# amcpherson/defuse

Hardware: AMD Instinct MI355X
Metric: split-read DP aligns/sec (higher is better)
Workload: dtype int16

## Files before the change

defuse_amd/csrc/dsa_kernels.hpp:

```cpp
#pragma once
#include <hip/hip_runtime.h>
#include <stdint.h>

#include "../../include/defuse_dsa.h"
#include "dsa_diag.hpp"
#include "dsa_tile.hpp"

namespace dsa {

constexpr int W = TILE_W;
constexpr int WAVE = 64;
constexpr int WG_WAVES = 4;
constexpr int WG_LANES = WG_WAVES * WAVE;
constexpr uint32_t REF_PAD16 = 0x00AAu;
constexpr uint32_t ROW_PAD16 = 0x0055u;

constexpr int NCLS = 5;
constexpr int NCOMBO = NCLS * NCLS;
constexpr int TROW = W + 4;
#ifndef FILL_PF
#define FILL_PF 2
#endif
constexpr int GMAX = 4;
constexpr int TGROUP = NCOMBO * TROW;
// ... 700 lines not shown
            ++gi;
        }
        tasks[tb + t] = rt;
    }
}

struct HitCursor {
    int k0, k1;
    int row0, row1;
    uint32_t t0, t1;
    uint64_t valid0, valid1;
};
__device__ __forceinline__ KeptRow kept_row(const KeptRow* __restrict__ kr, const uint64_t* kc, int k)
{
    if (kc != nullptr && k < KCACHE) return __builtin_bit_cast(KeptRow, kc[k * WG_LANES]);
    return kr[k];
}
__device__ __forceinline__ void cursor_next0(HitCursor& hc, const KeptRow* __restrict__ kr, const uint64_t* kc, int n_kept, bool has0)
{
    hc.row0 = -1;
    if (has0 && hc.k0 < n_kept) {
        const KeptRow r = kept_row(kr, kc, hc.k0);
        hc.row0 = r.a;
        hc.t0 = (uint32_t)(r.m1 + 2 * r.a) + BIAS16;
    }
}
__device__ __forceinline__ void cursor_next1(HitCursor& hc, const KeptRow* __restrict__ kr, const uint64_t* kc, int lq, bool has1)
{
    hc.row1 = -1;
    if (has1 && hc.k1 >= 0) {
        const KeptRow r = kept_row(kr, kc, hc.k1);
        hc.row1 = lq - r.a;
        hc.t1 = (uint32_t)(r.m2 + 2 * (lq - r.a)) + BIAS16;
    }
}
__device__ __forceinline__ HitCursor cursor_init(const KeptRow* __restrict__ kr, const uint64_t* kc, int n_kept, int lq,
                                                 bool has0, bool has1, int nv0, int nv1)
{
    HitCursor hc;
    hc.k0 = 0;
    hc.k1 = n_kept - 1;
    hc.t0 = hc.t1 = 0;
    hc.valid0 = nv0 >= W ? ~0ull : ((1ull << (nv0 > 0 ? nv0 : 0)) - 1ull);
    hc.valid1 = nv1 >= W ? ~0ull : ((1ull << (nv1 > 0 ? nv1 : 0)) - 1ull);
    cursor_next0(hc, kr, kc, n_kept, has0);
    cursor_next1(hc, kr, kc, lq, has1);
    return hc;
}

constexpr uint32_t NO_TARGET16 = 0x7F00u;
template <int WT>
__device__ __forceinline__ void equal_columns(const uint32_t (&X)[WT], uint32_t target2, uint64_t& m0, uint64_t& m1)
{
    uint32_t hit[W / 16];
    const uint32_t below = target2 - 0x00010001u;
#pragma unroll
    for (int q = 0; q < W / 16; ++q) {
        uint32_t acc = 0;
#pragma unroll
        for (int k = 15; k >= 0; --k) {
            const int i = 16 * q + k;
            if (i >= WT) continue;
            const uint32_t c = below + drift2(i);
            typedef unsigned short us2 __attribute__((ext_vector_type(2)));
            const uint32_t y = __builtin_bit_cast(uint32_t, __builtin_elementwise_sub_sat(__builtin_bit_cast(us2, X[i]), __builtin_bit_cast(us2, c)));
            asm("v_lshl_or_b32 %0, %0, 1, %1" : "+v"(acc) : "v"(y));
        }
        hit[q] = acc;
    }
    const uint32_t lo_a = (hit[0] & 0xFFFFu) | (hit[1] << 16), lo_b = (hit[2] & 0xFFFFu) | (hit[3] << 16);
    const uint32_t hi_a = (hit[0] >> 16) | (hit[1] & 0xFFFF0000u), hi_b = (hit[2] >> 16) | (hit[3] & 0xFFFF0000u);
    m0 = (uint64_t)lo_a | ((uint64_t)lo_b << 32);
    m1 = (uint64_t)hi_a | ((uint64_t)hi_b << 32);
}

template <int WT>
__device__ __forceinline__ void record_hits(const uint32_t (&X)[WT], int j, int lq, const KeptRow* __restrict__ kr,
                                            const uint64_t* kc, int n_kept, bool has0, bool has1, HitCursor& hc,
                                            uint64_t* __restrict__ masks, uint32_t mask_begin)
{
    const bool hit0 = hc.row0 == j, hit1 = hc.row1 == j;
    if (!(hit0 || hit1)) return;
    uint64_t m0, m1;
    equal_columns(X, (hit0 ? hc.t0 : NO_TARGET16) | ((hit1 ? hc.t1 : NO_TARGET16) << 16), m0, m1);
    if (hit0) {
        masks[((uint64_t)mask_begin + hc.k0) * 2] = m0 & hc.valid0;
        ++hc.k0;
        cursor_next0(hc, kr, kc, n_kept, has0);
    }
    if (hit1) {
        masks[((uint64_t)mask_begin + hc.k1) * 2 + 1] = m1 & hc.valid1;
        --hc.k1;
        cursor_next1(hc, kr, kc, lq, has1);
    }
}

__device__ __forceinline__ int64_t count_one_tile_pair(const uint64_t* mk, int n_kept)
{
    int64_t n = 0;
    for (int k = 0; k < n_kept; ++k) {
        const uint64_t m0 = mk[2 * k], m1 = mk[2 * k + 1];
        if (k == 0) {
            n += (int64_t)__builtin_popcountll(m0) * __builtin_popcountll(m1);
            continue;
        }
        for (uint64_t r0 = m0; r0; r0 &= r0 - 1)
            for (uint64_t r1 = m1; r1; r1 &= r1 - 1) {
                const int i1 = __builtin_ctzll(r0), i2 = __builtin_ctzll(r1);
                bool dup = false;
                for (int k2 = 0; k2 < k && !dup; ++k2) dup = ((mk[2 * k2] >> i1) & 1ull) && ((mk[2 * k2 + 1] >> i2) & 1ull);
                n += dup ? 0 : 1;
            }
    }
    return n;
}

template <bool SPLIT, int WT>
__device__ __forceinline__ void replay_fast_wg(uint32_t* T, FinishLds* fl, const WgView& wgi, const FinishBufs& fb,
                                               const uint32_t* __restrict__ refcodes, const uint32_t* __restrict__ rowcodes,
                                               const uint32_t* __restrict__ bnd, const Geom& g)
{
    const KeptRow* __restrict__ kept = fb.kept;
    uint64_t* __restrict__ masks = fb.masks;
    bool any = false;
    for (int k = 0; k < wgi.n_groups; ++k) any |= fl->tile[k] >= 0;
    if (!uniform(any)) return;
    build_tables<SPLIT, WT>(T, wgi.n_groups, [&](int gi, int i, uint32_t& q0, uint32_t& q1) {
        const int key = fl->tile[gi];
        q0 = q1 = REF_PAD16;
        if (key >= 0) {
            const int c0 = key >> 8, c1 = key & 0xFF;
            const uint32_t* rc = refcodes + (int64_t)group_fusion(wgi, gi) * g.lrp;
            if (c0 != NO_CHUNK) q0 = rc[c0 * W + i] & 0xFFFFu;
            if (c1 != NO_CHUNK) q1 = rc[c1 * W + i] >> 16;
        }
    });
    for (int e = threadIdx.x; e < 258; e += WG_LANES) fl->hist[e] = 0;
    __syncthreads();
    int my_key = 256, my_rank = 0;
    {
        const LaneInfo mine = fl->info[threadIdx.x];
        if (mine.last_row & TASK_FAST) my_key = mine.key_group & 0xFF;
        my_rank = atomicAdd(&fl->hist[my_key], 1);
    }
    __syncthreads();
    if (threadIdx.x == 0) {
        int run = 0;
        for (int e = 0; e < 257; ++e) {
            const int n = fl->hist[e];
            fl->hist[e] = run;
            run += n;
        }
    }
    __syncthreads();
    fl->order[fl->hist[my_key] + my_rank] = (unsigned short)threadIdx.x;
    __syncthreads();

    const int src = fl->order[threadIdx.x];
    const LaneInfo li = fl->info[src];
    const int64_t p = (int64_t)blockIdx.x * WG_LANES + src;
    const int lane = (int)(p & 63);
    const int64_t w = p >> 6;
    const bool has = (li.last_row & TASK_FAST) != 0;
    const int R = has ? (li.last_row & TASK_ROW) : 0;
    int Rw = R;
#pragma unroll
    for (int d = 32; d >= 1; d >>= 1) Rw = max(Rw, __shfl_xor(Rw, d, 64));
    Rw = uniform(Rw);
    if (Rw == 0) return;
    const bool has0 = has && li.c0 != NO_CHUNK, has1 = has && li.c1 != NO_CHUNK;
    const int c0 = has0 ? li.c0 : 0, c1 = has1 ? li.c1 : 0;
    const uint32_t* tb = T + (li.key_group >> 8) * (SPLIT ? TGROUP_SPLIT : TGROUP);
    const int64_t wr = w < g.n_waves ? w : (int64_t)blockIdx.x * WG_WAVES;
    const uint4* rows4 = reinterpret_cast<const uint4*>(rowcodes + wr * g.lq1 * WAVE) + lane;
    const uint4* bi0 = reinterpret_cast<const uint4*>(bnd + (wr * g.nch + (c0 - 1)) * g.lq1 * WAVE) + lane;
    const uint4* bi1 = reinterpret_cast<const uint4*>(bnd + (wr * g.nch + (c1 - 1)) * g.lq1 * WAVE) + lane;
    const KeptRow* kr = kept + li.kept_begin;
    const uint64_t* kc = fl->kc + src;
    const int lq = li.lq;
    const int n_kept = has ? li.n_kept : 0;
    HitCursor hc = cursor_init(kr, kc, n_kept, lq, has0, has1, li.nv0, li.nv1);
    const int stop0 = c0 > 0 ? load_tstop(fb.tstop + wr * g.nch + (c0 - 1)) : 0;
    const int stop1 = c1 > 0 ? load_tstop(fb.tstop + wr * g.nch + (c1 - 1)) : 0;

    uint32_t X[WT];
#pragma unroll
    for (int i = 0; i < WT; ++i) X[i] = BIAS2 + drift2(i);
    const uint4 bias4 = make_uint4(BIAS2, BIAS2, BIAS2, BIAS2);
    uint32_t bprev = BIAS2;
    const int ngq = (Rw >> 2) + 1;
    auto boundary = [&](int gq) -> uint4 {
        uint4 x0 = bias4, x1 = bias4;
        if (gq < stop0) x0 = load_group(bi0 + (int64_t)gq * WAVE);
        if (gq < stop1) x1 = load_group(bi1 + (int64_t)gq * WAVE);
        return make_uint4((x0.x & 0xFFFFu) | (x1.x & 0xFFFF0000u), (x0.y & 0xFFFFu) | (x1.y & 0xFFFF0000u),
                          (x0.z & 0xFFFFu) | (x1.z & 0xFFFF0000u), (x0.w & 0xFFFFu) | (x1.w & 0xFFFF0000u));
    };
    uint4 rc_n = rows4[0];
    uint4 b_n = boundary(0);
    for (int gq = 0; gq < ngq; ++gq) {
        const uint4 rc = rc_n, b = b_n;
        const int gn = gq + 1 < ngq ? gq + 1 : gq;
        rc_n = rows4[(int64_t)gn * WAVE];
        b_n = boundary(gn);
        const uint32_t rcv[4] = {rc.x, rc.y, rc.z, rc.w}, bv[4] = {b.x, b.y, b.z, b.w};
#pragma unroll
        for (int sidx = 0; sidx < 4; ++sidx) {
            const int j = 4 * gq + sidx;
            const uint32_t bcur = bv[sidx];
            if (j >= 1 && j <= Rw) {
                const uint4* trow = reinterpret_cast<const uint4*>(tb + (rcv[sidx] & 0xFFu) * TROW);
                auto table4 = [&](int q) -> uint4 {
                    if (SPLIT) return split_terms(tb, (rcv[sidx] >> 16) & 0xFu, (rcv[sidx] >> 20) & 0xFu, q);
                    return trow[q];
                };
                uint4 v = table4(0);
                uint32_t a = bprev + v.x;
                uint32_t up = bcur - TWO2;
#pragma unroll
                for (int q = 0; q < WT / 4; ++q) {
                    uint4 vn = v;
                    if (q + 1 < WT / 4) vn = table4(q + 1);
                    uint32_t an;
                    an = X[4 * q + 0] + v.y;
                    X[4 * q + 0] = max3(a, X[4 * q + 0], up);
                    a = an;
                    an = X[4 * q + 1] + v.z;
                    X[4 * q + 1] = max3(a, X[4 * q + 1], X[4 * q + 0]);
                    a = an;
                    an = X[4 * q + 2] + v.w;
                    X[4 * q + 2] = max3(a, X[4 * q + 2], X[4 * q + 1]);
                    a = an;
                    an = X[4 * q + 3] + vn.x;
                    X[4 * q + 3] = max3(a, X[4 * q + 3], X[4 * q + 2]);
                    a = an;
                    up = X[4 * q + 3];
                    v = vn;
                }
                record_hits(X, j, lq, kr, kc, n_kept, has0, has1, hc, masks, li.mask_begin);
            }
            bprev = bcur;
        }
    }
    if (has && !has0)
        for (int k = 0; k < n_kept; ++k) masks[((uint64_t)li.mask_begin + k) * 2] = 0;
    if (has && !has1)
        for (int k = 0; k < n_kept; ++k) masks[((uint64_t)li.mask_begin + k) * 2 + 1] = 0;
    if (has && (li.last_row & TASK_ONLY) && p < g.n_pairs)
        fb.rec_count[g.orig ? g.orig[p] : p] = count_one_tile_pair(masks + (uint64_t)li.mask_begin * 2, n_kept);
}

template <bool MASKED, int WT>
__device__ __forceinline__ int sweep_tile_generic(const uint32_t (&r)[WT], const uint4* __restrict__ rows4,
                                                  const uint4* __restrict__ bi4, uint4* __restrict__ cm4,
                                                  uint4* __restrict__ bo4, int lq, bool first, int nv0, int nv1,
                                                  int lq_lane, int slack, int l_in, int stop_prev, int& last_bnd)
{
    uint32_t X[WT];
#pragma unroll
    for (int i = 0; i < WT; ++i) X[i] = BIAS2 + drift2(i);
    const uint4 bias4 = make_uint4(BIAS2, BIAS2, BIAS2, BIAS2);
    uint32_t bprev = BIAS2;
    const int ngq = (lq >> 2) + 1;
    uint4 rc_n = rows4[0];
    uint4 b_n = first ? bias4 : bi4[0];
    last_bnd = 0;
    int gq = 0;
    for (; gq < ngq; ++gq) {
        const uint4 rc = rc_n, b = b_n;
        const int gn = gq + 1 < ngq ? gq + 1 : gq;
        rc_n = rows4[(int64_t)gn * WAVE];
        b_n = (!first && gn < stop_prev) ? bi4[(int64_t)gn * WAVE] : bias4;
        const uint32_t rcv[4] = {rc.x, rc.y, rc.z, rc.w}, bv[4] = {b.x, b.y, b.z, b.w};
        uint32_t cmv[4] = {BIAS2, BIAS2, BIAS2, BIAS2}, bov[4] = {BIAS2, BIAS2, BIAS2, BIAS2};
        bool alive = false;
#pragma unroll
        for (int sidx = 0; sidx < 4; ++sidx) {
            const int j = 4 * gq + sidx;
            if (j >= 1 && j <= lq) {
                row_step(X, r, rcv[sidx], bprev, bv[sidx]);
                cmv[sidx] = tile_row_max<MASKED>(X, nv0, nv1);
                bov[sidx] = X[WT - 1] - drift2(WT - 1);
                const int thr = 4 * j - slack + (int)BIAS16;
                const bool in_read = j <= lq_lane;
                alive |= in_read && ((int)(cmv[sidx] & 0xFFFFu) >= thr || (int)(cmv[sidx] >> 16) >= thr);
                if (in_read && ((int)(bov[sidx] & 0xFFFFu) >= thr || (int)(bov[sidx] >> 16) >= thr)) last_bnd = j;
            }
            bprev = bv[sidx];
        }
        cm4[(int64_t)gq * WAVE] = make_uint4(cmv[0], cmv[1], cmv[2], cmv[3]);
        bo4[(int64_t)gq * WAVE] = make_uint4(bov[0], bov[1], bov[2], bov[3]);
        if (DIAG_PRUNE && 4 * gq + 3 > l_in && __builtin_amdgcn_ballot_w64(alive) == 0) { ++gq; break; }
    }
    return gq;
}

__device__ __forceinline__ void max4(uint4& m, const uint4& v)
{
    m.x = max2(m.x, v.x);
    m.y = max2(m.y, v.y);
    m.z = max2(m.z, v.z);
    m.w = max2(m.w, v.w);
}
template <bool WIDE>
__device__ __forceinline__ void reduce_row_max(const uint32_t* __restrict__ cmax, uint32_t* __restrict__ rmax,
                                               const int32_t* tstop, const TileStops& stops,
                                               const Geom& g, int w, int lane, int nch_wave, int lq)
{
    const int ngq = (lq >> 2) + 1;
    const uint4 dead4 = make_uint4(BIAS2, BIAS2, BIAS2, BIAS2);
    uint4* out = reinterpret_cast<uint4*>(rmax + (int64_t)w * g.lq1 * WAVE) + lane;
    const uint4* src = reinterpret_cast<const uint4*>(cmax + (int64_t)w * g.nch * g.lq1 * WAVE) + lane;
    const int64_t cstride = (int64_t)(g.lq1 >> 2) * WAVE;
    constexpr int NC = 8;
    if (nch_wave <= NC) {
        for (int gq = 0; gq < ngq; ++gq) {
            uint4 v[NC];
#pragma unroll
            for (int c = 0; c < NC; ++c)
                if (gq < stops.v[c]) v[c] = src[c * cstride + (int64_t)gq * WAVE];
            uint4 m = dead4;
#pragma unroll
            for (int c = 0; c < NC; ++c)
                if (gq < stops.v[c]) max4(m, v[c]);
            out[(int64_t)gq * WAVE] = m;
        }
        return;
    }
    if (WIDE && nch_wave <= 2 * NC) {
        int stop_hi[NC];
#pragma unroll
        for (int c = 0; c < NC; ++c) stop_hi[c] = NC + c < nch_wave ? uniform(load_tstop(tstop + (int64_t)w * g.nch + NC + c)) : 0;
        for (int gq = 0; gq < ngq; ++gq) {
            uint4 v[NC], u[NC];
#pragma unroll
            for (int c = 0; c < NC; ++c) {
                if (gq < stops.v[c]) v[c] = src[c * cstride + (int64_t)gq * WAVE];
                if (gq < stop_hi[c]) u[c] = src[(NC + c) * cstride + (int64_t)gq * WAVE];
            }
            uint4 m = dead4;
#pragma unroll
            for (int c = 0; c < NC; ++c) {
                if (gq < stops.v[c]) max4(m, v[c]);
                if (gq < stop_hi[c]) max4(m, u[c]);
            }
            out[(int64_t)gq * WAVE] = m;
        }
        return;
    }
    for (int gq = 0; gq < ngq; ++gq) {
        uint4 m = dead4;
        for (int c = 0; c < nch_wave; ++c)
            if (gq < uniform(load_tstop(tstop + (int64_t)w * g.nch + c))) max4(m, src[c * cstride + (int64_t)gq * WAVE]);
        out[(int64_t)gq * WAVE] = m;
    }
}

template <int WT>
__global__ __launch_bounds__(WG_LANES) void k_fill_generic(const dsa_pair* __restrict__ pairs,
                                                           const dsa_fusion* __restrict__ fusions,
                                                           const uint8_t* __restrict__ wg_tier,
                                                           const uint32_t* __restrict__ refcodes,
                                                           const uint8_t* __restrict__ read_bytes,
                                                           uint32_t* __restrict__ rowcodes,
                                                           const int32_t* __restrict__ min_score_tab,
                                                           uint32_t* __restrict__ bnd, uint32_t* __restrict__ cmax,
                                                           uint32_t* __restrict__ rmax,
                                                           FinishBufs fb, Geom g)
{
    __shared__ FinishLds fl;
    if (wg_tier[blockIdx.x] != TIER_GENERIC) return;
    if (threadIdx.x == 0) atomicAdd(&fb.ctr->fill_wgs[FILL_WGS_GENERIC], 1u);
    const int w = __builtin_amdgcn_readfirstlane((int)(blockIdx.x * WG_WAVES + (threadIdx.x >> 6)));
    TileStops stops = {};
    if (w < g.n_waves) {
        const int lane = threadIdx.x & 63;
        const int64_t p = min((int64_t)w * WAVE + lane, g.n_pairs - 1);
        const bool in_batch = (int64_t)w * WAVE + lane < g.n_pairs;
        const int f = pairs[p].fusion_idx;
        const dsa_fusion fu = fusions[f];
        auto wave_max = [](int v) {
#pragma unroll
            for (int d = 32; d >= 1; d >>= 1) v = max(v, __shfl_xor(v, d, 64));
            return uniform(v);
        };
        WaveInfo wi;
        wi.lq_max = wave_max(in_batch ? (int)pairs[p].read_len : 0);
        wi.nch_max = wave_max(in_batch ? max(cdiv_dev(fu.ref0_len, WT), cdiv_dev(fu.ref1_len, WT)) : 0);
        (void)pack_rows_wave<0>(read_bytes, pairs, rowcodes, nullptr, g, w, lane, wi.lq_max);
        const uint32_t* rc = refcodes + (int64_t)f * g.lrp;
        const uint4* rows4 = reinterpret_cast<const uint4*>(rowcodes + (int64_t)w * g.lq1 * WAVE) + lane;
        int lq_lane = 0, slack = 0;
        if (in_batch) {
            lq_lane = pairs[p].read_len;
            slack = 2 * lq_lane - max(min_score_tab[lq_lane], pair_bound(pairs[p]));
        }
        int l_in = wave_max(lq_lane > 0 ? min(slack >> 2, lq_lane) : 0);
        int stop_prev = 0;

        for (int c = 0; c < wi.nch_max; ++c) {
            uint32_t r[WT];
#pragma unroll
            for (int i = 0; i < WT; ++i) r[i] = rc[c * W + i];
            const int nv0 = fu.ref0_len - c * WT, nv1 = fu.ref1_len - c * WT;
            uint4* cm4 = reinterpret_cast<uint4*>(cmax + ((int64_t)w * g.nch + c) * g.lq1 * WAVE) + lane;
            uint4* bo4 = reinterpret_cast<uint4*>(bnd + ((int64_t)w * g.nch + c) * g.lq1 * WAVE) + lane;
            const uint4* bi4 = reinterpret_cast<const uint4*>(bnd + ((int64_t)w * g.nch + (c - 1)) * g.lq1 * WAVE) + lane;
            int last_bnd, stop;
            if (__builtin_amdgcn_ballot_w64(nv0 < WT || nv1 < WT) == 0)
                stop = sweep_tile_generic<false, WT>(r, rows4, bi4, cm4, bo4, wi.lq_max, c == 0, nv0, nv1, lq_lane, slack, l_in, stop_prev, last_bnd);
            else
                stop = sweep_tile_generic<true, WT>(r, rows4, bi4, cm4, bo4, wi.lq_max, c == 0, nv0, nv1, lq_lane, slack, l_in, stop_prev, last_bnd);
            if (lane == 0) fb.tstop[(int64_t)w * g.nch + c] = stop;
            stop_prev = stop;
#pragma unroll
            for (int k = 0; k < 8; ++k)
                if (k == c) stops.v[k] = stop;
            l_in = wave_max(last_bnd);
        }
        __builtin_amdgcn_fence(__ATOMIC_RELEASE, "workgroup");
        reduce_row_max<false>(cmax, rmax, fb.tstop, stops, g, w, lane, wi.nch_max, wi.lq_max);
    }
    WgView wgi = {};
    wgi.list = nullptr;
    combine_wg<false, WT>(pairs, fusions, cmax, rmax, stops, min_score_tab, wgi, 0, false, &fl, fb, g);
}

template <int NW, bool SPLIT, bool LAST>
__device__ __forceinline__ int sweep_tile_fast(const uint32_t* __restrict__ tb, const uint32_t* __restrict__ rows1, const uint4* __restrict__ bi4,
                                               uint4* __restrict__ cm4, uint4* __restrict__ bo4, bool first_tile, int lq_max, int lq_lane,
                                               uint32_t thr0, int l_in, int stop_prev, int& last_bnd, const Geom& g, int tile)
{
    static_assert(NW % 4 == 0 && NW / 4 > FILL_PF && NW <= W, "table reads in flight");
    (void)g; (void)tile;
    uint32_t X[NW];
#pragma unroll
    for (int i = 0; i < NW; ++i) X[i] = BIAS2 + drift2(i);
    const uint4 bias4 = make_uint4(BIAS2, BIAS2, BIAS2, BIAS2);
    uint32_t bprev = BIAS2;
    const int ngq = (lq_max >> 2) + 1;
    uint32_t rc_n = rows1[0];
    uint4 b_n = first_tile ? bias4 : bi4[0];
    last_bnd = 0;
    int gq = 0;
    int n_gap_groups = 0;
    for (; gq < ngq; ++gq) {
        const uint32_t rc = rc_n;
        const uint4 b = b_n;
        const int gn = gq + 1 < ngq ? gq + 1 : gq;
        rc_n = rows1[(int64_t)gn * WAVE];
        b_n = bias4;
        if (gn < stop_prev) b_n = load_group(bi4 + (int64_t)gn * WAVE);
        const uint32_t bv[4] = {b.x, b.y, b.z, b.w};
        uint32_t cmv[4] = {BIAS2, BIAS2, BIAS2, BIAS2}, bov[4] = {BIAS2, BIAS2, BIAS2, BIAS2};
        uint32_t alive_bits = 0;
#pragma unroll
        for (int sidx = 0; sidx < 4; ++sidx) {
            const int j = 4 * gq + sidx;
            const uint32_t bcur = bv[sidx];
            if (j >= 1 && j <= lq_max) {
                if constexpr (SPLIT) {
                    const uint32_t k1 = (rc >> (8 * sidx)) & 0xFu, k2 = (rc >> (8 * sidx + 4)) & 0xFu;
                    uint4 v = split_terms(tb, k1, k2, 0);
                    uint32_t a = bprev + v.x;
                    uint32_t up = bcur - TWO2;
#pragma unroll
                    for (int q = 0; q < NW / 4; ++q) {
                        uint4 vn = v;
                        if (q + 1 < NW / 4) vn = split_terms(tb, k1, k2, q + 1);
                        uint32_t an;
                        an = X[4 * q + 0] + v.y;
                        X[4 * q + 0] = max3(a, X[4 * q + 0], up);
                        a = an;
                        an = X[4 * q + 1] + v.z;
                        X[4 * q + 1] = max3(a, X[4 * q + 1], X[4 * q + 0]);
                        a = an;
                        an = X[4 * q + 2] + v.w;
                        X[4 * q + 2] = max3(a, X[4 * q + 2], X[4 * q + 1]);
                        a = an;
                        an = X[4 * q + 3] + vn.x;
                        X[4 * q + 3] = max3(a, X[4 * q + 3], X[4 * q + 2]);
                        a = an;
                        up = X[4 * q + 3];
                        v = vn;
                    }
                } else {
                    const uint4* trow = reinterpret_cast<const uint4*>(tb + ((rc >> (8 * sidx)) & 0xFFu) * TROW);
                    uint4 vq[FILL_PF + 1];
#pragma unroll
                    for (int k = 0; k <= FILL_PF; ++k) vq[k] = trow[k];
                    uint32_t a = bprev + vq[0].x;
                    uint32_t up = bcur - TWO2;
#pragma unroll
                    for (int q = 0; q < NW / 4; ++q) {
                        const uint4 v = vq[0];
#pragma unroll
                        for (int k = 0; k < FILL_PF; ++k) vq[k] = vq[k + 1];
                        if (q + 1 + FILL_PF < NW / 4) vq[FILL_PF] = trow[q + 1 + FILL_PF];
                        const uint4 vn = vq[0];
                        uint32_t an;
                        an = X[4 * q + 0] + v.y;
                        X[4 * q + 0] = max3(a, X[4 * q + 0], up);
                        a = an;
                        an = X[4 * q + 1] + v.z;
                        X[4 * q + 1] = max3(a, X[4 * q + 1], X[4 * q + 0]);
                        a = an;
                        an = X[4 * q + 2] + v.w;
                        X[4 * q + 2] = max3(a, X[4 * q + 2], X[4 * q + 1]);
                        a = an;
                        an = X[4 * q + 3] + vn.x;
                        X[4 * q + 3] = max3(a, X[4 * q + 3], X[4 * q + 2]);
                        a = an;
                        up = X[4 * q + 3];
                    }
                }
                {
                    uint32_t acc0 = BIAS2, acc1 = BIAS2;
#pragma unroll
                    for (int i = 0; i < NW; i += 4) {
                        acc0 = max3(acc0, X[i] - drift2(i), X[i + 1] - drift2(i + 1));
                        acc1 = max3(acc1, X[i + 2] - drift2(i + 2), X[i + 3] - drift2(i + 3));
                    }
                    cmv[sidx] = max2(acc0, acc1);
                }
                const uint32_t tm2 = thr_of_row(thr0, j, j <= lq_lane);
                alive_bits |= pk_max_u16(cmv[sidx], tm2) ^ tm2;
                if (!LAST) {
                    bov[sidx] = X[NW - 1] - drift2(NW - 1);
                    if ((pk_max_u16(bov[sidx], tm2) ^ tm2) != 0u) last_bnd = j;
                }
            }
            bprev = bcur;
        }
        const bool alive = alive_bits != 0u;
        cm4[(int64_t)gq * WAVE] = make_uint4(cmv[0], cmv[1], cmv[2], cmv[3]);
        if (!LAST) bo4[(int64_t)gq * WAVE] = make_uint4(bov[0], bov[1], bov[2], bov[3]);
        if (DIAG_PRUNE && __builtin_amdgcn_ballot_w64(alive) == 0) {
            if (4 * gq + 3 > l_in) { ++gq; break; }
            if (DIAG_GAP_SKIP) {
                int g2 = gq + 1;
                bool resume = false;
                uint4 bb = b_n;
                uint32_t in_prev = bv[3];
                for (; g2 < ngq; ++g2) {
                    if (g2 > gq + 1) {
                        bb = bias4;
                        if (g2 < stop_prev) bb = load_group(bi4 + (int64_t)g2 * WAVE);
                    }
                    const uint32_t bbv[5] = {in_prev, bb.x, bb.y, bb.z, bb.w};
                    uint32_t in_bits = 0;
#pragma unroll
                    for (int sidx = 0; sidx < 5; ++sidx) {
                        const int j = 4 * g2 + sidx - 1;
                        const uint32_t tm2 = thr_of_row(thr0, j, j <= lq_lane);
                        in_bits |= pk_max_u16(bbv[sidx], tm2) ^ tm2;
                    }
                    if (__builtin_amdgcn_ballot_w64(in_bits != 0u) != 0) { resume = true; break; }
                    cm4[(int64_t)g2 * WAVE] = bias4;
                    if (!LAST) bo4[(int64_t)g2 * WAVE] = bias4;
                    in_prev = bb.w;
                    if (4 * g2 + 3 > l_in) { ++g2; break; }
                }
                n_gap_groups += g2 - (gq + 1);
                if (!resume) { gq = g2; break; }
#pragma unroll
                for (int i = 0; i < NW; ++i) X[i] = BIAS2 + drift2(i);
                bprev = in_prev;
                b_n = bb;
                rc_n = rows1[(int64_t)g2 * WAVE];
                gq = g2 - 1;
            }
        }
    }
    if ((threadIdx.x & 63) == 0) {
        DSA_STAT_ADD(g, DS_GAP_GROUPS, n_gap_groups);
        DSA_STAT_ADD(g, DS_GROUPS_SKIPPED, ngq - gq);
        DSA_STAT_ADD(g, DS_GROUPS, ngq);
        DSA_STAT_ADD(g, DS_TILE_GROUPS + (tile < DS_TILE_SLOTS ? tile : DS_TILE_SLOTS - 1), gq - n_gap_groups);
    }
    return gq;
}

__host__ __device__ constexpr int tier_of(int n_groups) { return n_groups <= GMAX ? 0 : n_groups <= GSPLIT ? 1 : 2; }
#ifndef DSA_FAST_WGS
#define DSA_FAST_WGS 4
#endif
template <int TIER, bool WIDE, int WT>
__global__ __launch_bounds__(WG_LANES, TIER == 2 ? 2 : DSA_FAST_WGS) void k_fill_fast(const dsa_pair* __restrict__ pairs,
                                                           uint8_t* __restrict__ wg_tier,
                                                           const uint32_t* __restrict__ refcodes,
                                                           const uint8_t* __restrict__ read_bytes,
                                                           uint32_t* __restrict__ rowcodes, uint32_t* __restrict__ row_bytes,
                                                           const int32_t* __restrict__ min_score_tab,
                                                           const dsa_fusion* __restrict__ fusions,
                                                           uint32_t* __restrict__ bnd, uint32_t* __restrict__ cmax,
                                                           uint32_t* __restrict__ rmax,
                                                           FinishBufs fb, Geom g)
{
    constexpr bool SPLIT = TIER > 0;
    __shared__ __attribute__((aligned(16))) uint32_t T[TIER == 2 ? GSPLIT2 * TGROUP_SPLIT : GMAX * TGROUP];
    __shared__ int s_nch, s_exotic;
    __shared__ FinishLds fl;
    __shared__ WgGroupsLds gl;
    if (TIER != 0 && wg_tier[blockIdx.x] != TIER) return;
    const int w = __builtin_amdgcn_readfirstlane((int)(blockIdx.x * WG_WAVES + (threadIdx.x >> 6)));
    const bool live = w < g.n_waves;
    const int lane = threadIdx.x & 63;
    const int64_t p = (int64_t)w * WAVE + lane;
    const bool in_batch = p < g.n_pairs;
    const dsa_pair pr = pairs[min(p, g.n_pairs - 1)];
    const int f = pr.fusion_idx;
    int my_group;
    const WgView wgi = wg_groups(&gl, f, (lane == 0 && threadIdx.x != 0) ? pairs[min(p - 1, g.n_pairs - 1)].fusion_idx : -1, my_group);
    if (TIER == 0) {
        const int tier = wgi.n_groups == 0 ? (int)TIER_GENERIC : tier_of(wgi.n_groups);
        if (threadIdx.x == 0) {
            wg_tier[blockIdx.x] = (uint8_t)tier;
            if (tier != 0) atomicOr(&fb.ctr->need_tiers, 1u << tier);
        }
        if (tier != 0) return;
    }
    int lq_lane = 0, slack = 0, tiles_lane = 0;
    if (in_batch) {
        const dsa_fusion fu = fusions[f];
        lq_lane = pr.read_len;
        slack = 2 * lq_lane - max(min_score_tab[lq_lane], pair_bound(pr));
        tiles_lane = max(cdiv_dev(fu.ref0_len, WT), cdiv_dev(fu.ref1_len, WT));
    }
    auto wave_max = [](int v) {
#pragma unroll
        for (int d = 32; d >= 1; d >>= 1) v = max(v, __shfl_xor(v, d, 64));
        return uniform(v);
    };
    WaveInfo wi;
    wi.lq_max = wave_max(lq_lane);
    wi.nch_max = wave_max(tiles_lane);
    int l_in = wave_max(lq_lane > 0 ? min(slack >> 2, lq_lane) : 0);
    const bool exotic = live && pack_rows_wave<SPLIT ? 2 : 1>(read_bytes, pairs, rowcodes, row_bytes, g, w, lane, wi.lq_max);
    if (threadIdx.x == 0) { s_nch = 0; s_exotic = 0; }
    __syncthreads();
    if (lane == 0 && live) atomicMax(&s_nch, wi.nch_max);
    if (__builtin_amdgcn_ballot_w64(exotic) != 0 && lane == 0) atomicOr(&s_exotic, 1);
    __syncthreads();
    if (uniform(s_exotic) != 0) {
        if (threadIdx.x == 0) {
            wg_tier[blockIdx.x] = TIER_GENERIC;
            atomicOr(&fb.ctr->need_tiers, 1u << TIER_GENERIC);
        }
        return;
    }
// ... 612 lines not shown
```

Measured before the change: 326.5 million.

## Software-pipeline row-max reduction loads with branchless alive-tile substitution

Rewrites the per-row column-max reduction so that every one of the eight per-chunk loads is issued without a branch. A chunk that has already stopped reads from the longest-lived chunk's tile instead, which leaves the max unchanged. Loads are multi-buffered across RMAX_SETS row groups (and double-buffered in the wide path) so memory latency overlaps the max3 folds. Rows past the longest stop are written directly as dead values. The trade-off is extra register pressure from holding several sets of uint4 loads, plus redundant loads for dead chunks.

```diff
diff --git a/defuse_amd/csrc/dsa_kernels.hpp b/defuse_amd/csrc/dsa_kernels.hpp
--- a/defuse_amd/csrc/dsa_kernels.hpp
+++ b/defuse_amd/csrc/dsa_kernels.hpp
@@ -1026,6 +1026,9 @@
     m.z = max2(m.z, v.z);
     m.w = max2(m.w, v.w);
 }
+#ifndef RMAX_SETS
+#define RMAX_SETS 3
+#endif
 template <bool WIDE>
 __device__ __forceinline__ void reduce_row_max(const uint32_t* __restrict__ cmax, uint32_t* __restrict__ rmax,
                                                const int32_t* tstop, const TileStops& stops,
@@ -1037,39 +1040,74 @@
     const uint4* src = reinterpret_cast<const uint4*>(cmax + (int64_t)w * g.nch * g.lq1 * WAVE) + lane;
     const int64_t cstride = (int64_t)(g.lq1 >> 2) * WAVE;
     constexpr int NC = 8;
+    const char* planes = reinterpret_cast<const char*>(cmax + (int64_t)w * g.nch * g.lq1 * WAVE);
+    const int64_t tile_bytes = cstride * (int64_t)sizeof(uint4);
+    auto issue = [&](uint4 (&v)[NC], const int (&st)[NC], int c0, int gq, const char* alive_tile) {
+        const uint32_t at = (uint32_t)(gq * WAVE + lane) * (uint32_t)sizeof(uint4);
+#pragma unroll
+        for (int c = 0; c < NC; ++c) {
+            const char* tile = gq < st[c] ? planes + (c0 + c) * tile_bytes : alive_tile;
+            v[c] = load_group(reinterpret_cast<const uint4*>(tile + at));
+        }
+    };
+    auto fold = [](uint4& m, const uint4 (&v)[NC]) {
+#pragma unroll
+        for (int c = 0; c < NC; c += 2) {
+            m.x = max3(m.x, v[c].x, v[c + 1].x);
+            m.y = max3(m.y, v[c].y, v[c + 1].y);
+            m.z = max3(m.z, v[c].z, v[c + 1].z);
+            m.w = max3(m.w, v[c].w, v[c + 1].w);
+        }
+    };
+    auto longest = [](const int (&st)[NC], int c0, int& smax, int& cbest) {
+#pragma unroll
+        for (int c = 0; c < NC; ++c)
+            if (st[c] > smax) { smax = st[c]; cbest = c0 + c; }
+    };
     if (nch_wave <= NC) {
-        for (int gq = 0; gq < ngq; ++gq) {
-            uint4 v[NC];
-#pragma unroll
-            for (int c = 0; c < NC; ++c)
-                if (gq < stops.v[c]) v[c] = src[c * cstride + (int64_t)gq * WAVE];
-            uint4 m = dead4;
-#pragma unroll
-            for (int c = 0; c < NC; ++c)
-                if (gq < stops.v[c]) max4(m, v[c]);
-            out[(int64_t)gq * WAVE] = m;
-        }
+        int smax = 0, cbest = 0;
+        longest(stops.v, 0, smax, cbest);
+        smax = smax < ngq ? smax : ngq;
+        const char* alive_tile = planes + cbest * tile_bytes;
+        uint4 v[RMAX_SETS][NC];
+        if (smax > 0) {
+#pragma unroll
+            for (int d = 0; d < RMAX_SETS - 1; ++d) issue(v[d], stops.v, 0, d < smax ? d : smax - 1, alive_tile);
+        }
+        for (int g0 = 0; g0 < smax; g0 += RMAX_SETS) {
+#pragma unroll
+            for (int d = 0; d < RMAX_SETS; ++d) {
+                const int gq = g0 + d, ahead = gq + RMAX_SETS - 1;
+                if (gq >= smax) break;
+                issue(v[(d + RMAX_SETS - 1) % RMAX_SETS], stops.v, 0, ahead < smax ? ahead : smax - 1, alive_tile);
+                uint4 m = dead4;
+                fold(m, v[d]);
+                out[(int64_t)gq * WAVE] = m;
+            }
+        }
+        for (int gq = smax; gq < ngq; ++gq) out[(int64_t)gq * WAVE] = dead4;
         return;
     }
     if (WIDE && nch_wave <= 2 * NC) {
         int stop_hi[NC];
 #pragma unroll
         for (int c = 0; c < NC; ++c) stop_hi[c] = NC + c < nch_wave ? uniform(load_tstop(tstop + (int64_t)w * g.nch + NC + c)) : 0;
-        for (int gq = 0; gq < ngq; ++gq) {
-            uint4 v[NC], u[NC];
-#pragma unroll
-            for (int c = 0; c < NC; ++c) {
-                if (gq < stops.v[c]) v[c] = src[c * cstride + (int64_t)gq * WAVE];
-                if (gq < stop_hi[c]) u[c] = src[(NC + c) * cstride + (int64_t)gq * WAVE];
-            }
+        int smax = 0, cbest = 0;
+        longest(stops.v, 0, smax, cbest);
+        longest(stop_hi, NC, smax, cbest);
+        smax = smax < ngq ? smax : ngq;
+        const char* alive_tile = planes + cbest * tile_bytes;
+        uint4 va[NC], vb[NC];
+        if (smax > 0) issue(va, stops.v, 0, 0, alive_tile);
+        for (int gq = 0; gq < smax; ++gq) {
+            issue(vb, stop_hi, NC, gq, alive_tile);
             uint4 m = dead4;
-#pragma unroll
-            for (int c = 0; c < NC; ++c) {
-                if (gq < stops.v[c]) max4(m, v[c]);
-                if (gq < stop_hi[c]) max4(m, u[c]);
-            }
+            fold(m, va);
+            issue(va, stops.v, 0, gq + 1 < smax ? gq + 1 : gq, alive_tile);
+            fold(m, vb);
             out[(int64_t)gq * WAVE] = m;
         }
+        for (int gq = smax; gq < ngq; ++gq) out[(int64_t)gq * WAVE] = dead4;
         return;
     }
     for (int gq = 0; gq < ngq; ++gq) {
```

New measurement: 330.1 million (median of 6 runs). +1.1%, better.
